# bjack205/altro

Hardware: AMD Instinct MI355X
Metric: iLQR backward+forward sweeps/sec (N knotpoints x batch) (higher is better)
Workload: dtype f64

## Files before the change

### altro_amd/__init__.py

```python
import ctypes as C
import os

import numpy as np

_HERE = os.path.dirname(os.path.abspath(__file__))
LIB_PATH = os.path.join(_HERE, "lib", "libaltro_hip.so")

F64, F32 = 0, 1
PLAN_AUTO, PLAN_GENERIC, PLAN_MFMA16, PLAN_LANE, PLAN_MFMA32 = 0, 1, 2, 3, 4
STORE_QBLOCKS = 0x1
LANE_FUSED = 0x4
F32_PURE = 0x2
TILE_USER_BLOCKS = 0x2
GENERIC_MATRIX_CORES = 0x8
TVLQR_SUCCESS = -1

C_ABI_SYMBOLS = [
    "altro_hip_version", "altro_hip_last_error", "altro_hip_device_count", "altro_hip_device_info", "altro_hip_device_pci_bus_id",
    "altro_hip_batch_create", "altro_hip_batch_create_dims", "altro_hip_batch_destroy", "altro_hip_batch_plan",
    "altro_hip_batch_device_bytes", "altro_hip_set_dynamics", "altro_hip_set_cost",
    "altro_hip_set_initial_state", "altro_hip_set_host_batch", "altro_hip_backward", "altro_hip_forward_ltv", "altro_hip_sweep",
    "altro_hip_synchronize", "altro_hip_get_K", "altro_hip_get_d", "altro_hip_get_P",
    "altro_hip_get_p", "altro_hip_get_x", "altro_hip_get_u", "altro_hip_get_y",
    "altro_hip_get_delta_V", "altro_hip_get_status", "altro_hip_get_qblocks",
    "altro_hip_stats_reduce", "altro_hip_comm_unique_id", "altro_hip_comm_create", "altro_hip_comm_create_all",
    "altro_hip_comm_destroy", "altro_hip_comm_rank", "altro_hip_comm_world", "altro_hip_comm_device", "altro_hip_stats_allreduce", "altro_hip_stats_allreduce_multi",
    "altro_hip_profile_enable", "altro_hip_profile_reset",
    "altro_hip_profile_get", "altro_hip_profile_get_range", "altro_hip_profile_dropped", "altro_hip_algorithmic_bytes",
    "altro_hip_set_model", "altro_hip_set_model_source", "altro_hip_model_row_layout", "altro_hip_set_tracking_cost", "altro_hip_set_quadratic_cost",
    "altro_hip_set_input_guess", "altro_hip_set_state_guess",
    "altro_hip_open_loop_rollout", "altro_hip_accept", "altro_hip_expand", "altro_hip_merit",
    "altro_hip_stationarity", "altro_hip_get_nominal", "altro_hip_get_expansion",
    "altro_hip_default_solve_options", "altro_hip_set_forms", "altro_hip_get_forms", "altro_hip_ilqr_solve", "altro_hip_last_solve_counts",
    "altro_hip_ilqr_solve_async", "altro_hip_ilqr_poll", "altro_hip_ilqr_wait",
    "altro_hip_linesearch_host",
    "altro_hip_add_linear_constraint", "altro_hip_add_user_constraint", "altro_hip_clear_constraints", "altro_hip_reset_duals",
    "altro_hip_get_duals", "altro_hip_set_duals", "altro_hip_get_penalty", "altro_hip_set_penalty", "altro_hip_shift_duals", "altro_hip_feasibility",
    "altro_hip_shift_trajectory", "altro_hip_update_linear_costs", "altro_hip_get_knot",
    "altro_hip_set_pointer_mode",
]
CONE_EQUALITY, CONE_IDENTITY, CONE_INEQUALITY, CONE_SOC = 0, 1, 2, 3

DUAL_TAIL_KEEP, DUAL_TAIL_ZERO = 0, 1
FORM_NO_SPECULATION, FORM_NO_RUNAHEAD, FORM_NO_MERIT2, FORM_MERIT_LDS, FORM_MERIT_DPP_ALWAYS = 0x1, 0x2, 0x4, 0x8, 0x10
FORM_EXPAND_LDS, FORM_ALROWS_LDS, FORM_ROLLOUT_ROUNDS, FORM_SEQUENCED, FORM_MERIT_ONE_LAUNCH = 0x20, 0x40, 0x80, 0x100, 0x200
FORM_LANE_QUAD_OFF, FORM_LANE_QUAD_ON, FORM_GENERIC_LATE_Q_OFF, FORM_GENERIC_LATE_Q_ON, FORM_FUSED_CLOCK = 0x400, 0x800, 0x1000, 0x2000, 0x4000
FORM_AFFINE_EXACT = 0x8000
FORM_NO_COMPACTION = 0x10000
FORM_GENERIC_MERIT_LDS = 0x20000


def forms_from_env():
    e = os.environ
    off = lambda name: e.get(name) is not None and e[name].strip() not in ("",) and _atoi(e[name]) == 0
    f = 0
    if "ALTRO_HIP_NO_SPECULATION" in e: f |= FORM_NO_SPECULATION
    if "ALTRO_HIP_NO_RUNAHEAD" in e and not off("ALTRO_HIP_NO_RUNAHEAD"): f |= FORM_NO_RUNAHEAD
    if off("ALTRO_HIP_MERIT2"): f |= FORM_NO_MERIT2
    if off("ALTRO_HIP_MERIT_DPP"): f |= FORM_MERIT_LDS
    elif e.get("ALTRO_HIP_MERIT_DPP") is not None and _atoi(e["ALTRO_HIP_MERIT_DPP"]) == 2: f |= FORM_MERIT_DPP_ALWAYS
    if off("ALTRO_HIP_EXPAND_DPP"): f |= FORM_EXPAND_LDS
    if off("ALTRO_HIP_ALROWS_DPP"): f |= FORM_ALROWS_LDS
    if off("ALTRO_HIP_AFFINE"): f |= FORM_ROLLOUT_ROUNDS
    if off("ALTRO_HIP_FUSED") or "ALTRO_HIP_NO_FUSED" in e: f |= FORM_SEQUENCED
    if off("ALTRO_HIP_MERIT_SPLIT"): f |= FORM_MERIT_ONE_LAUNCH
    if "ALTRO_HIP_LANE_QUAD" in e: f |= FORM_LANE_QUAD_OFF if _atoi(e["ALTRO_HIP_LANE_QUAD"]) == 0 else FORM_LANE_QUAD_ON
    if "ALTRO_HIP_GENERIC_LATE_Q" in e: f |= FORM_GENERIC_LATE_Q_OFF if _atoi(e["ALTRO_HIP_GENERIC_LATE_Q"]) == 0 else FORM_GENERIC_LATE_Q_ON
    if "ALTRO_HIP_FUSED_CLOCK" in e: f |= FORM_FUSED_CLOCK
    if "ALTRO_HIP_AFFINE_EXACT" in e: f |= FORM_AFFINE_EXACT
    if "ALTRO_HIP_NO_COMPACTION" in e: f |= FORM_NO_COMPACTION
    return f


def _atoi(text):
    try:
        return int(text.strip() or 0)
    except ValueError:
        return 0

MODEL_LINEAR, MODEL_DOUBLE_INTEGRATOR, MODEL_PENDULUM, MODEL_BICYCLE, MODEL_USER, MODEL_QUADROTOR, MODEL_QUADROTOR13 = 0, 1, 2, 3, 4, 5, 6
MERIT_FN = C.CFUNCTYPE(None, C.c_double, C.POINTER(C.c_double), C.POINTER(C.c_double), C.c_void_p)


class SolveOptions(C.Structure):
    _fields_ = [("iterations_max", C.c_int), ("tol_stationarity", C.c_double),
                ("tol_primal_feasibility", C.c_double), ("tol_meritfun_gradient", C.c_double),
                ("use_backtracking_linesearch", C.c_int), ("penalty_initial", C.c_double),
                ("penalty_scaling", C.c_double), ("penalty_max", C.c_double), ("reg_initial", C.c_double),
                ("reg_retry_max", C.c_int), ("reg_scale", C.c_double), ("reg_min", C.c_double),
                ("reg_max", C.c_double), ("stop_when_running_at_most", C.c_int),
                ("forms", C.c_uint), ("fused_sweeps", C.c_int), ("decision_margin", C.c_double)]


class SolveResult(C.Structure):
    _fields_ = [("status", C.c_int), ("iterations", C.c_int), ("stationarity", C.c_double),
                ("final_alpha", C.c_double), ("final_phi", C.c_double), ("primal_feasibility", C.c_double),
                ("penalty", C.c_double), ("dual_updates", C.c_int), ("reg_retries", C.c_int)]


class PollRecord(C.Structure):
    _fields_ = [("result", SolveResult), ("u0", C.c_double * 4), ("done", C.c_int), ("reserved", C.c_int)]


class AltroHipError(RuntimeError):
    pass


class Stats(C.Structure):
    _fields_ = [("problems", C.c_int64), ("cholesky_failures", C.c_int64), ("converged", C.c_int64),
                ("iterations", C.c_int64), ("sum_cost", C.c_double),
                ("sum_delta_V0", C.c_double), ("sum_delta_V1", C.c_double),
                ("max_stationarity", C.c_double), ("max_feasibility", C.c_double), ("max_abs_xN", C.c_double),
                ("non_finite", C.c_int64)]
    SUM_FIELDS = ("problems", "cholesky_failures", "converged", "iterations", "sum_cost", "sum_delta_V0", "sum_delta_V1",
                  "non_finite")
    MAX_FIELDS = ("max_stationarity", "max_feasibility", "max_abs_xN")

    def as_dict(self):
        return {k: getattr(self, k) for k, _ in self._fields_}


COMM_ID_BYTES = 128

# ... 516 lines not shown
```

### altro_amd/csrc/capi_ilqr.hip

```cpp
#include "capi_internal.h"

#include <cstring>

using namespace altro_hip;
using namespace altro_hip::capi;

namespace altro_hip {
namespace capi {

static AlInput al_input(const altro_hip_batch* h) {
  return AlInput{h->plan, h->n, h->m, h->N, h->batch, h->dtype == ALTRO_HIP_F64 ? sizeof(double) : sizeof(float), h->ragged, h->nxv, h->nuv,
                 h->al_defs, h->al_knots, h->al_G, h->al_g};
}
static int al_copy(altro_hip_batch* h, void** dst, const void* src, size_t bytes) {
  if (const int rc = dmalloc(h, dst, bytes)) return rc;
  HIP_TRY(hipMemcpy(*dst, src, bytes, hipMemcpyHostToDevice));
  return 0;
}
static int al_copy_pool(altro_hip_batch* h, void** dst, const std::vector<double>& pool) {
  if (h->dtype == ALTRO_HIP_F64) return al_copy(h, dst, pool.data(), pool.size() * sizeof(double));
  const std::vector<float> f = al_pool_as<float>(pool);
  return al_copy(h, dst, f.data(), f.size() * sizeof(float));
}
static int al_upload_tables(altro_hip_batch* h) {
// ... 124 lines not shown
    const RouteStep& st = route.step[i];
    a.mode = st.mode; a.mp.kind = st.kind;
    if (st.rtc) {
      if (!module_current) {
        if (const int rc = rtc_current(h, shape)) return rc;
        module_current = true;
      }
      if (const int rc = rtc_step(h, st, &a)) return rc;
      continue;
    }
    const int rc = launch_step(h, st, a);
    if (rc == 1) return fail(ALTRO_HIP_ERR_UNSUPPORTED, "internal error: kernel %#x is not in its launcher unit", st.id);
    if (rc) return fail(ALTRO_HIP_ERR_HIP, "iLQR kernel launch failed");
  }
  return 0;
}
template <typename T>
int lane_run(altro_hip_batch* h, int which, bool use_alpha, bool use_active, int want_deriv, double alpha_const, int mode) {
  const IlqrArgs<T> a = ilqr_args<T>(h, use_alpha, use_active, want_deriv, alpha_const);
  const RouteShape shape = route_shape(h);
  const Route route = loop_route(shape, RouteCall{which, mode, a.spec_trials});
  if (route.error == ROUTE_NO_MODEL) return fail(ALTRO_HIP_ERR_UNSUPPORTED, "no device model for (kind, n, m) = (%d, %d, %d)", h->model.kind, h->n, h->m);
  if (route.error) return fail(ALTRO_HIP_ERR_UNSUPPORTED, "operation %d is not available on plan LANE", which);
  return route_execute(h, shape, route, a);
}
template <typename S>
int wave_run(altro_hip_batch* h, int which, bool use_alpha, bool use_active, int want_deriv, double alpha_const, int mode) {
  IlqrWaveArgs<S> a;
  a.al = al_table<S>(h);
  a.mode = mode;
  const bool user_al = a.al.enabled && h->al_sum.has_user;
  if (user_al && (h->forms & (ALTRO_HIP_FORM_MERIT_LDS | ALTRO_HIP_FORM_ALROWS_LDS | ALTRO_HIP_FORM_EXPAND_LDS)))
    return fail(ALTRO_HIP_ERR_UNSUPPORTED, "constraint blocks from source on plan MFMA16 run in the row-layout kernels only: the LDS comparison forms "
                                           "(ALTRO_HIP_FORM_MERIT_LDS, _ALROWS_LDS, _EXPAND_LDS) do not evaluate them");
  a.penalty_scaling = h->expand_penalty_scaling; a.penalty_max = h->expand_penalty_max;
  a.costd = (const S*)h->m_costd; a.costd_term = (const S*)h->m_costd_term; a.cost_dense = h->cost_dense ? 1 : 0;
  if (h->model_set) a.mp = h->model;
  a.dyn = (const S*)h->m_in; a.dyn_bs = h->m_st.in_bs; a.dyn_ks = h->m_st.in_ks;
  a.cin = (S*)h->m_cin; a.cin_bs = h->m_st.cin_bs; a.cin_ks = h->m_st.cin_ks;
  a.term = (S*)h->m_term; a.out = (const S*)h->m_out; a.out_bs = h->m_st.out_bs; a.out_ks = h->m_st.out_ks;
  a.outn = (const S*)h->m_outn; a.nom = (S*)h->m_nom; a.cand = (S*)h->m_xuy; a.xuy_bs = h->m_st.xuy_bs;
  a.xuy_ks = h->m_st.xuy_ks; a.costp = (const S*)h->m_costp; a.x0 = (const S*)h->x0;
  a.alpha = use_alpha ? h->i_alpha : nullptr; a.active = use_active ? h->i_active : nullptr;
  a.phi = h->i_phi; a.dphi = h->i_dphi; a.prob = h->i_prob; a.N = h->N; a.batch = h->batch;
  a.want_derivative = want_deriv; a.alpha_const = alpha_const;
  a.cand_spec = (S*)h->i_cand_spec; a.spec_trials = h->i_cand_spec ? h->spec_trials : 1; a.spec_sel = h->i_spec_sel;
  a.spec_pre = h->i_cand_spec ? h->spec_pre : 0;
  a.spec_stride = (int64_t)h->batch * (h->N + 1) * MF_XUY;
  a.ls_beta = h->spec_beta; a.ls_max_iters = h->spec_max_iters;
  a.skip = which == IK_STATIONARITY ? h->stat_skip : nullptr;
  const bool aff_on = sizeof(S) == 8 && h->aff_enabled && !h->model_set;
  const bool aff_store = aff_on && h->aff_store && (which == IK_MERIT2 || which == IK_MERIT);
  const RouteShape shape = route_shape(h);
  const Route route = loop_route(shape, RouteCall{which, mode, a.spec_trials, aff_on && !aff_store && which == IK_MERIT && h->aff_round && !a.spec_pre});
  if (route.error) return fail(ALTRO_HIP_ERR_UNSUPPORTED, "operation %d is not available on plan MFMA16", which);
  if constexpr (sizeof(S) == 8) {
    a.aff = route.count && (route.step[0].id & KF_AFF) ? 1 : 0;
    if (aff_store || a.aff) { a.sens = (double*)h->i_sens; a.sens_alpha = (double*)h->i_sens_alpha; }
    if (a.aff) { a.aff_part = (double*)h->i_aff_part; a.aff_on = (int*)h->i_aff_on; }
  }
  return route_execute(h, shape, route, a);
}
struct GenSizes { int64_t sx, su, sQ, sR, sH; };
GenSizes gen_sizes(const altro_hip_batch* h) {
  GenSizes z{0, 0, 0, 0, 0};
  for (int k = 0; k <= h->N; ++k) {
    const int64_t nk = h->ragged ? h->nxv[k] : h->n, mk = k < h->N ? (h->ragged ? h->nuv[k] : h->m) : 0;
    z.sx += nk; z.su += mk; z.sQ += nk * nk; z.sR += mk * mk; z.sH += mk * nk;
  }
  return z;
}
template <typename T>
int gen_run(altro_hip_batch* h, int which, bool use_alpha, bool use_active, int want_deriv, double alpha_const, int mode) {
  const int n = h->n, m = h->m, N = h->N;
  IlqrGenArgs<T> a;
  a.A = (const T*)h->g_arr[G_A]; a.A_bs = h->g_bstride[G_A]; a.B = (const T*)h->g_arr[G_B]; a.B_bs = h->g_bstride[G_B];
  a.f = (const T*)h->g_arr[G_f]; a.f_bs = h->g_bstride[G_f];
  a.Q = (T*)h->g_arr[G_Q]; a.Q_bs = h->g_bstride[G_Q]; a.R = (T*)h->g_arr[G_R]; a.R_bs = h->g_bstride[G_R];
  a.H = (T*)h->g_arr[G_H]; a.H_bs = h->g_bstride[G_H]; a.q = (T*)h->g_arr[G_q]; a.q_bs = h->g_bstride[G_q];
  a.r = (T*)h->g_arr[G_r]; a.r_bs = h->g_bstride[G_r];
  a.K = (const T*)h->g_arr[G_K]; a.K_bs = h->g_bstride[G_K]; a.d = (const T*)h->g_arr[G_d]; a.d_bs = h->g_bstride[G_d];
  a.P = (const T*)h->g_arr[G_P]; a.P_bs = h->g_bstride[G_P]; a.p = (const T*)h->g_arr[G_p]; a.p_bs = h->g_bstride[G_p];
  a.x = (T*)h->g_arr[G_x]; a.x_bs = h->g_bstride[G_x]; a.u = (T*)h->g_arr[G_u]; a.u_bs = h->g_bstride[G_u];
  a.y = (T*)h->g_arr[G_y]; a.y_bs = h->g_bstride[G_y];
  a.xn = (T*)h->g_xn; a.un = (T*)h->g_un;
  a.cQ = (const T*)h->g_cQ; a.cR = (const T*)h->g_cR; a.cH = (const T*)h->g_cH; a.cq = (const T*)h->g_cq; a.cr = (const T*)h->g_cr;
  a.cc = (const T*)h->g_cc;
  a.x0 = (const T*)h->x0; a.x0_stride = h->x0_stride;
  a.alpha = use_alpha ? h->i_alpha : nullptr; a.active = use_active ? h->i_active : nullptr; a.alpha_const = alpha_const;
  a.phi = h->i_phi; a.dphi = h->i_dphi; a.prob = h->i_prob;
  a.N = N; a.n = n; a.m = m; a.batch = h->batch; a.want_derivative = want_deriv; a.mode = mode;
  a.off = h->g_off; a.nx = h->g_nx; a.nu = h->g_nu;
  const GenSizes gs = gen_sizes(h);
  a.sx = gs.sx; a.su = gs.su; a.sQ = gs.sQ; a.sR = gs.sR; a.sH = gs.sH;
  a.al = al_table<T>(h);
  const RouteShape shape = route_shape(h);
  a.row32 = row32_eligible(shape) ? 1 : 0;
  a.row32m = row32_model_eligible(shape) ? 1 : 0;
  if ((a.row32 || a.row32m) && which == IK_STATIONARITY && N > R32_STAT_CHUNK) {
    const size_t need = (size_t)((N + R32_STAT_CHUNK - 1) / R32_STAT_CHUNK) * h->batch * 2 * sizeof(double);
    if (h->g_stat_part_bytes < need) {
      if (h->g_stat_part) { (void)hipFree(h->g_stat_part); h->g_stat_part = nullptr; h->g_stat_part_bytes = 0; }
      if (hipMalloc((void**)&h->g_stat_part, need) == hipSuccess) h->g_stat_part_bytes = need;
      else { (void)hipGetLastError(); h->g_stat_part = nullptr; }
    }
    a.stat_part = h->g_stat_part;
  }
// ... 802 lines not shown
```

### altro_amd/csrc/ilqr_launch_mfma16.hip

```cpp
#include <hip/hip_runtime.h>

#include "kernels/ilqr_mfma16.hip"
#include "kernels/ilqr_merit2_dpp.hip"
#include "loop_route.h"

namespace altro_hip {

using namespace capi;

#define GO(...) hipLaunchKernelGGL((__VA_ARGS__), grid, block, st.lds, stream, a); break
#define MERIT(DUAL_, DENSE_, AFF_)                                                                                              \
  case merit_id(true, DUAL_, DENSE_, false, AFF_): GO(wave_merit_dpp_kernel<S, true, DUAL_, DENSE_, 0, false, AFF_>);           \
  case merit_id(true, DUAL_, DENSE_, true, AFF_): GO(wave_merit_dpp_kernel<S, true, DUAL_, DENSE_, 0, true, AFF_>);             \
  case merit_id(false, DUAL_, DENSE_, true, AFF_): GO(wave_merit_dpp_kernel<S, false, DUAL_, DENSE_, 0, true, AFF_>)

template <typename S>
static int wave_launch(hipStream_t stream, const RouteStep& st, const IlqrWaveArgs<S>& a) {
  const dim3 grid(st.gx, st.gy, st.gz), block(st.block);
  if constexpr (sizeof(S) == 8) {
    if ((st.id & KF_AFF) || st.id == K_WAVE_AFF_REDUCE) {
      switch (st.id) {
        MERIT(false, false, true);
        MERIT(false, true, true);
        case K_WAVE_AFF_REDUCE: hipLaunchKernelGGL(wave_aff_reduce_kernel<S>, grid, block, 0, stream, a, st.chunks); break;
        default: return 1;
      }
      return hipGetLastError() == hipSuccess ? 0 : 2;
    }
  }
  switch (st.id) {
    case K_WAVE_ROLLOUT: GO(wave_rollout_kernel<S>);
    case K_WAVE_ACCEPT: GO(wave_accept_kernel<S>);
    case K_WAVE_EXPAND_DPP | KF_DENSE: GO(wave_expand_dpp_kernel<S, true>);
    case K_WAVE_EXPAND_DPP | KF_ALLSEL: GO(wave_expand_dpp_kernel<S, false, true>);
    case K_WAVE_EXPAND_DPP: GO(wave_expand_dpp_kernel<S, false>);
    case K_WAVE_EXPAND_LDS: GO(wave_expand_kernel<S>);
    case K_WAVE_EXPAND_GRAD | KF_DENSE: GO(wave_expand_grad_dense_kernel<S>);
    case K_WAVE_EXPAND_GRAD: GO(wave_expand_grad_kernel<S>);
    case K_WAVE_DUAL_DPP: GO(wave_dual_update_dpp_kernel<S>);
    case K_WAVE_DUAL_LDS: GO(wave_dual_update_kernel<S>);
    MERIT(false, false, false);
    MERIT(false, true, false);
    MERIT(true, false, false);
    MERIT(true, true, false);
    case K_WAVE_MERIT_LDS | KF_AL: GO(wave_merit_kernel<S, true>);
    case K_WAVE_MERIT_LDS: GO(wave_merit_kernel<S, false>);
    case K_WAVE_SPEC_SELECT: GO(wave_spec_select_kernel<S>);
    case K_WAVE_STATIONARITY: GO(wave_stationarity_kernel<S>);
    case K_WAVE_FEAS_DPP: GO(wave_feasibility_dpp_kernel<S>);
    case K_WAVE_SHIFT: GO(wave_shift_kernel<S>);
    default: return 1;
  }
  return hipGetLastError() == hipSuccess ? 0 : 2;
}
#undef MERIT
#undef GO
template <>
int ilqr_wave_launch_kernel<double>(hipStream_t stream, const RouteStep& st, const IlqrWaveArgs<double>& a) { return wave_launch<double>(stream, st, a); }
template <>
int ilqr_wave_launch_kernel<float>(hipStream_t stream, const RouteStep& st, const IlqrWaveArgs<float>& a) { return wave_launch<float>(stream, st, a); }

}
```

### altro_amd/csrc/kernels/ilqr_merit2_dpp.hip

```cpp
#pragma once

namespace altro_hip {

constexpr int MD_ZLD = 18;
constexpr int MD_OUT0 = 12 * MD_ZLD;
constexpr int MD_F0 = MD_OUT0 + MF_OUT;
constexpr int MD_NOM0 = MD_F0 + 12;
constexpr int MD_CP0 = MD_NOM0 + MF_NOM;
constexpr int MD_IMG = MD_CP0 + MF_COSTP;
constexpr int MD_IMG_DENSE = MD_CP0 + MF_COST;
static_assert(MF_DYN % 2 == 0 && MF_OUT % 2 == 0 && MF_NOM % 2 == 0 && MF_COSTP % 2 == 0 && MD_IMG % 2 == 0, "records move as pairs");

typedef double md_d2 __attribute__((ext_vector_type(2)));
typedef float md_f2 __attribute__((ext_vector_type(2)));
template <typename S> struct md_pair_of;
template <> struct md_pair_of<double> { typedef md_d2 type; };
template <> struct md_pair_of<float> { typedef md_f2 type; };
template <typename S>
__device__ __forceinline__ md_d2 md_ld(const S* __restrict__ p, int pair) {
  const typename md_pair_of<S>::type v = *reinterpret_cast<const typename md_pair_of<S>::type*>(p + 2 * pair);
  return md_d2{(double)v[0], (double)v[1]};
}
template <bool DENSE = false>
struct MeritPairRegs { md_d2 z[3], f, o[3], nm, cp[DENSE ? 3 : 1]; };
// ... 1008 lines not shown
      else a.cin[(size_t)b * a.cin_bs + (size_t)k * a.cin_ks + MF_OFF_HR + (r - 12) * 16 + j] = (S)v;
    }
  }
}

template <typename S>
__global__ __launch_bounds__(64) void wave_dual_update_dpp_kernel(IlqrWaveArgs<S> a) {
  const int lane = threadIdx.x, j = lane & 15;
  const int wpk = (a.batch + 3) >> 2;
  const int k = (int)(blockIdx.x / wpk), b0 = (int)(blockIdx.x % wpk) * 4, b_own = b0 + (lane >> 4);
  if (k > a.N || !a.al.enabled) return;
  const bool on = b_own < a.batch && a.prob[b_own < a.batch ? b_own : 0].dual != 0;
  const unsigned long long onm = __ballot(on);
  if (onm == 0ull) return;
  const int b = on ? b_own : b0 + (__builtin_ctzll(onm) >> 4);
  const bool terminal = k == a.N;
  const S* c = a.cand + (size_t)b * a.xuy_bs + (size_t)k * a.xuy_ks;
  const double w = j < 12 ? (double)c[j] : (terminal ? 0.0 : (double)c[12 + j]);
  double jvr[AL_TILE_MAXC], cost = 0.0, viol = 0.0;
#ifdef MD_USER_BLOCKS
  __shared__ double uimg[4][MD_UIMG_ROW];
  dpp_al_rows<S, true>(a.al, k, b, a.batch, w, terminal, a.prob[b].rho_est, j, jvr, cost, viol, on, uimg[lane >> 4]);
#else
  dpp_al_rows<S, true>(a.al, k, b, a.batch, w, terminal, a.prob[b].rho_est, j, jvr, cost, viol, on);
#endif
}
template <typename S>
__global__ __launch_bounds__(64) void wave_feasibility_dpp_kernel(IlqrWaveArgs<S> a) {
  const int lane = threadIdx.x, j = lane & 15;
  const int wpk = (a.batch + 3) >> 2;
  const int k = (int)(blockIdx.x / wpk), b0 = (int)(blockIdx.x % wpk) * 4, b_own = b0 + (lane >> 4);
  if (k > a.N) return;
  bool on = b_own < a.batch;
  if (on && a.active && !a.active[b_own]) on = false;
  if (on && a.skip && a.skip[b_own]) on = false;
  const unsigned long long onm = __ballot(on);
  if (onm == 0ull) return;
  const int b = on ? b_own : b0 + (__builtin_ctzll(onm) >> 4);
  const bool terminal = k == a.N;
  const S* c = a.cand + (size_t)b * a.xuy_bs + (size_t)k * a.xuy_ks;
  const double w = j < 12 ? (double)c[j] : (terminal ? 0.0 : (double)c[12 + j]);
  double jvr[AL_TILE_MAXC], cost = 0.0, viol = 0.0;
#ifdef MD_USER_BLOCKS
  __shared__ double uimg[4][MD_UIMG_ROW];
  dpp_al_rows<S>(a.al, k, b, a.batch, w, terminal, a.prob[b].rho, j, jvr, cost, viol, false, uimg[lane >> 4]);
#else
  dpp_al_rows<S>(a.al, k, b, a.batch, w, terminal, a.prob[b].rho, j, jvr, cost, viol);
#endif
#pragma unroll
  for (int o = 8; o > 0; o >>= 1) viol = fmax(viol, __shfl_xor(viol, o, 64));
  if (j == 0 && on && viol > 0.0)
    atomicMax(reinterpret_cast<unsigned long long*>(&a.prob[b].feasibility), (unsigned long long)__double_as_longlong(viol));
}


}
```

### altro_amd/csrc/loop_route.h

```cpp
#pragma once
#include <algorithm>
#include <cstdint>

#include "al_tables.h"
#include "kernels/ilqr_types.h"
#include "rtc_unit.h"

namespace altro_hip {
namespace capi {

enum KernelId : int {
  KF_AL = 1,
  KF_DUAL = 2,
  KF_DENSE = 4,
  KF_SOC = 8,
  KF_AFF = 16,
  KF_WIDE = 32,
  KF_MODEL = 64,
  KF_ALLSEL = 128,
  KF_STAGED = 128,
  KF_MASK = 255,
  K_WAVE_ROLLOUT = 1 << 8 , K_WAVE_ACCEPT = 2 << 8,
  K_WAVE_EXPAND_GRAD = 3 << 8,
  K_WAVE_EXPAND_DPP = 4 << 8 , K_WAVE_EXPAND_LDS = 5 << 8,
// ... 15 lines not shown
#define ILQR_LANE_MODELS(X)                                                                 \
  X(MODEL_PENDULUM, 2, 1) X(MODEL_BICYCLE, 4, 2) X(MODEL_DOUBLE_INTEGRATOR, 2, 1)           \
  X(MODEL_DOUBLE_INTEGRATOR, 4, 2) X(MODEL_DOUBLE_INTEGRATOR, 6, 3)
constexpr bool lane_model_supported(int kind, int n, int m) {
#define X(K_, N_, M_) if (kind == K_ && n == N_ && m == M_) return true;
  ILQR_LANE_MODELS(X)
#undef X
  return false;
}
constexpr int merit_id(bool al, bool dual, bool dense, bool soc, bool aff = false, int more = 0) {
  return K_WAVE_MERIT_DPP | (al ? KF_AL : 0) | (dual ? KF_DUAL : 0) | (dense ? KF_DENSE : 0) | (soc ? KF_SOC : 0) | (aff ? KF_AFF : 0) | more;
}
enum RouteUnit { RU_MFMA16, RU_MFMA16_MODEL, RU_MFMA16_WIDE, RU_LANE, RU_GENERIC, RU_ROW32 , RU_ROW32_MODEL };
constexpr int route_unit(int id) {
  return id >= K_LANE ? RU_LANE : id >= K_ROW_MERIT ? ((id & KF_MODEL) ? RU_ROW32_MODEL : RU_ROW32) : id >= K_GEN_ROLLOUT ? RU_GENERIC : (id & KF_WIDE) ? RU_MFMA16_WIDE : (id & KF_MODEL) ? RU_MFMA16_MODEL : RU_MFMA16;
}
constexpr int route_rtc_slot(int id) {
  if (id >= K_LANE) return (id - K_LANE) >> 8;
  switch (id & ~KF_MASK) {
    case K_WAVE_ROLLOUT: return RTT_ROLLOUT;
    case K_WAVE_EXPAND_DYN: return RTT_EXPAND_DYN;
    case K_WAVE_MERIT_DPP: return (id & KF_DUAL) ? RTT_MERIT2 : RTT_MERIT;
    case K_WAVE_EXPAND_DPP: return RTT_EXPAND_AL;
    case K_WAVE_DUAL_DPP: return RTT_DUAL;
    case K_WAVE_FEAS_DPP: return RTT_FEAS;
    case K_GEN_ROLLOUT: return RTG_ROLLOUT;
    case K_GEN_EXPAND_DYN: return RTG_EXPAND_DYN;
    case K_GEN_MERIT: return RTG_MERIT;
    case K_ROW_MERIT: return (id & KF_DUAL) ? RTG_ROW_MERIT2 : RTG_ROW_MERIT;
    case K_ROW_EXPAND_DYN: return RTG_ROW_EXPAND_DYN;
    case K_GEN_STATIONARITY: return RTG_STATIONARITY;
    case K_GEN_EXPAND_AL: return RTG_EXPAND_AL;
    case K_GEN_DUAL: return RTG_DUAL;
    default: return -1;
  }
}

struct RouteShape {
  int plan;
  bool f64, ragged;
  int n, m, N, batch;
  int model;
  bool cost_dense;
  bool merit_split;
  unsigned forms;
  bool al_enabled;
  AlSummary al;
  bool row_ok;
};
struct RouteCall {
  int which, mode, spec_trials;
  bool aff;
  bool stat_part;
};
enum RouteError { ROUTE_OK = 0, ROUTE_NO_KERNEL , ROUTE_NO_MODEL  };
struct RouteStep {
  bool rtc;
  int id;
  unsigned gx, gy, gz, block, lds;
  int mode, kind;
  int chunks;
};
constexpr int ROUTE_MAX_STEPS = 4;
struct Route {
  int error = ROUTE_OK, count = 0;
  RouteStep step[ROUTE_MAX_STEPS] = {};
};

inline unsigned route_merit_lds(const RouteShape& s, bool rtc) {
  if (!s.al_enabled) return 0u;
  const unsigned padded = (unsigned)s.al.Gpad_count * 8u;
  return rtc && s.al.has_user ? std::max(padded, (unsigned)AL_GP_DEF * 8u) : padded;
}
inline int route_tile_module_key(const RouteShape& s) {
  return (s.al_enabled ? 1 : 0) | (s.cost_dense ? 2 : 0) | ((s.al_enabled && s.al.max_ncon > AL_MAXC) ? 4 : 0) | ((s.al_enabled && s.al.has_user) ? 8 : 0);
}

inline Route route_mfma16(const RouteShape& s, const RouteCall& c) {
  Route r;
  const auto frm = [&](unsigned bit) { return (s.forms & bit) != 0; };
  const bool al = s.al_enabled, wide = al && s.al.max_ncon > AL_MAXC, model = s.model != MODEL_LINEAR, user = s.model == MODEL_USER;
  const bool user_al = user && al && s.al.has_user;
  const int dense = s.cost_dense ? KF_DENSE : 0;
  int mode = c.mode;
  if (c.which == IK_STATIONARITY || c.which == IK_DUAL) mode = frm(ALTRO_HIP_FORM_ALROWS_LDS) ? 0 : STAT_NO_FEAS;
  if (c.which == IK_EXPAND && frm(ALTRO_HIP_FORM_EXPAND_LDS) && !s.cost_dense) mode |= EXPAND_LDS;
  if (model && c.which == IK_EXPAND && (mode & EXPAND_GRADIENT) && !(mode & EXPAND_NEXT)) mode |= EXPAND_DYN;
  if (c.which == IK_MERIT) mode = frm(ALTRO_HIP_FORM_MERIT_LDS) ? 0 : frm(ALTRO_HIP_FORM_MERIT_DPP_ALWAYS) ? 3 : 2;
  const int lib_kind = user ? (int)MODEL_LINEAR : s.model;
  int rtc_kind = MODEL_USER;
  const auto add = [&](bool rtc, int id, int64_t gx, unsigned gy = 1, unsigned gz = 1, unsigned block = 64, unsigned lds = 0, int chunks = 0) {
    r.step[r.count++] = RouteStep{rtc, id, (unsigned)gx, gy, gz, block, lds, mode, rtc ? rtc_kind : lib_kind, chunks};
  };
  const auto no_kernel = [&] { r.error = ROUTE_NO_KERNEL; r.count = 0; return r; };
  if (model && (!s.f64 || (!user && s.model != MODEL_QUADROTOR))) return no_kernel();
  if (wide && !s.f64 && (c.which == IK_EXPAND || c.which == IK_MERIT || c.which == IK_MERIT2)) return no_kernel();
  const int64_t knots = (int64_t)s.N + 1, rows4 = (s.batch + 3) / 4, flat = ((int64_t)s.batch * knots * 16 + 255) / 256;
  const unsigned waves = (unsigned)mf_grid(s.batch), pairs = (unsigned)mf_grid((s.batch + 1) / 2);
  const unsigned trials = (unsigned)std::max(c.spec_trials, 1);
  switch (c.which) {
    case IK_ROLLOUT:
      if (model) add(user, K_WAVE_ROLLOUT | KF_MODEL, rows4);
      else add(false, K_WAVE_ROLLOUT, waves);
      break;
    case IK_ACCEPT: add(false, K_WAVE_ACCEPT, std::min<int64_t>(flat, 1 << 20), 1, 1, 256); break;
    case IK_EXPAND:
      if (model && (mode & EXPAND_DYN)) add(user, K_WAVE_EXPAND_DYN | KF_MODEL, rows4 * s.N);
      if (user_al) {
        add(true, K_WAVE_EXPAND_DPP | dense | (wide ? KF_WIDE : 0), rows4 * knots);
        break;
      }
      if (al && (wide || dense || !(mode & EXPAND_LDS))) add(false, K_WAVE_EXPAND_DPP | (wide ? KF_WIDE : 0) | (dense ? dense : s.al.all_sel ? KF_ALLSEL : 0), rows4 * knots);
      else if (al) add(false, K_WAVE_EXPAND_LDS, s.batch * knots);
      else if (mode & EXPAND_GRADIENT) add(false, K_WAVE_EXPAND_GRAD | dense, std::min<int64_t>(flat, 262144), 1, 1, 256);
      break;
    case IK_DUAL:
      if (user_al) { add(true, K_WAVE_DUAL_DPP, rows4 * knots); break; }
      if (mode & STAT_NO_FEAS) add(false, K_WAVE_DUAL_DPP, rows4 * knots);
      else add(false, K_WAVE_DUAL_LDS, s.batch * knots);
      break;
    case IK_MERIT:
    case IK_MERIT2: {
      const bool dual = c.which == IK_MERIT2, aff = !dual && !model && s.f64 && c.aff && mode >= 2;
      const unsigned gy = dual ? 1u : (trials + 1) / 2;
      if (!model && !wide && !dual && !aff && !dense && mode != 2 && mode != 3) {
        add(false, K_WAVE_MERIT_LDS | (al ? KF_AL : 0), waves, trials);
        break;
      }
      const int id = merit_id(al, dual, s.cost_dense, model || !al || s.al.has_soc, aff, (model ? KF_MODEL : 0) | (wide ? KF_WIDE : 0));
      if (aff) {
        const int chunks = (s.N + MD_AFF_CHUNK - 1) / MD_AFF_CHUNK;
        add(false, id, pairs, gy, (unsigned)chunks, 64, route_merit_lds(s, false));
        add(false, K_WAVE_AFF_REDUCE | (wide ? KF_WIDE : 0), ((int64_t)ILQR_SPEC_TRIALS * s.batch + 255) / 256, 1, 1, 256, 0, chunks);
      } else {
        add(user, id, pairs, gy, 1, 64, route_merit_lds(s, user));
      }
      break;
    }
    case IK_SPEC_SELECT: add(false, K_WAVE_SPEC_SELECT, s.batch); break;
    case IK_STATIONARITY:
      if (user_al) { mode |= STAT_FEAS_USER; rtc_kind = MODEL_LINEAR; }
      if (al && (mode & STAT_NO_FEAS)) {
        add(false, K_WAVE_STATIONARITY, waves);
        add(user_al, K_WAVE_FEAS_DPP, rows4 * knots);
      } else {
        mode &= ~STAT_NO_FEAS;
        add(false, K_WAVE_STATIONARITY, waves);
      }
      break;
    case IK_SHIFT: add(false, K_WAVE_SHIFT, ((int64_t)s.batch * 16 + 255) / 256, 1, 1, 256); break;
    default: return no_kernel();
  }
  return r;
}

inline Route route_lane(const RouteShape& s, const RouteCall& c) {
  Route r;
  const bool user = s.model == MODEL_USER;
  if (!user && !lane_model_supported(s.model, s.n, s.m)) { r.error = ROUTE_NO_MODEL; return r; }
  const auto add = [&](int slot, bool dense, int64_t gx, unsigned gy, unsigned block) {
    r.step[r.count++] = RouteStep{user, lane_id(slot, dense), (unsigned)gx, gy, 1, block, 0, c.mode, s.model, 0};
  };
  const int64_t total = (int64_t)s.batch * (s.N + 1), lanes = (s.batch + 63) / 64;
  const int64_t flat = std::min<int64_t>((total + 255) / 256, 1 << 20), flat64 = std::min<int64_t>((total + 63) / 64, 1 << 20);
  const unsigned trials = (unsigned)std::max(c.spec_trials, 1);
  switch (c.which) {
    case IK_ROLLOUT: add(RTC_ROLLOUT, false, lanes, 1, 64); break;
    case IK_ACCEPT: add(RTC_ACCEPT, false, flat, 1, 256); break;
    case IK_EXPAND: add(RTC_EXPAND, s.cost_dense, flat64, 1, 64); break;
    case IK_MERIT:
      if (s.merit_split) {
        add(RTC_MERIT_ROLL, false, lanes, trials, 64);
        add(RTC_MERIT_POINT, s.cost_dense, flat64, trials, 64);
        add(RTC_MERIT_SUM, false, lanes, trials, 64);
      } else {
        add(RTC_MERIT, s.cost_dense, lanes, trials, 64);
      }
      break;
    case IK_SPEC_SELECT: add(RTC_SPEC_SELECT, false, flat, 1, 256); break;
    case IK_DUAL: add(RTC_DUAL, false, flat, 1, 256); break;
    case IK_SHIFT: add(RTC_SHIFT, false, std::min<int64_t>(((int64_t)s.batch * (s.n + s.m) + 255) / 256, 1 << 20), 1, 256); break;
    case IK_STATIONARITY:
      add(RTC_ZERO_RESIDUALS, false, (s.batch + 255) / 256, 1, 256);
      add(RTC_STATIONARITY, false, flat64, 1, 64);
      break;
    default: r.error = ROUTE_NO_KERNEL;
  }
  return r;
}

constexpr bool tile32_shape_ok(int n, int m) { return n >= 5 && n <= T32_MAX_N && m >= 1 && m <= T32_MAX_M && n + m <= 32 && !(n <= 12 && m <= 4); }
constexpr bool gen_model_supported(int kind, int n, int m) { return kind == MODEL_QUADROTOR13 && n == 13 && m == 4; }
inline bool row32_shape(const RouteShape& s) {
  return s.plan == ALTRO_HIP_PLAN_GENERIC && s.f64 && !s.ragged && tile32_shape_ok(s.n, s.m) && !(s.forms & ALTRO_HIP_FORM_GENERIC_MERIT_LDS) && (!s.al_enabled || s.al.row32_ok);
}
inline bool row32_eligible(const RouteShape& s) { return row32_shape(s) && s.model == MODEL_LINEAR; }
inline bool row32_model_eligible(const RouteShape& s) {
// ... 19 lines not shown
  const int64_t b = s.batch, knots = (int64_t)s.N + 1, pairs = (b + 1) / 2, flat = std::min<int64_t>((b * knots * (s.n + s.m) + 255) / 256, 1 << 20);
  const unsigned jv = al ? (unsigned)(GEN_AL_JV * sizeof(double)) : 0u;
  switch (c.which) {
    case IK_ROLLOUT:
      if (user || q13) add(user, K_GEN_ROLLOUT | KF_MODEL, (b + 63) / 64);
      else if (row32 && (mode & ROLLOUT_INIT)) add(false, K_ROW_INIT, pairs);
      else add(false, K_GEN_ROLLOUT, b);
      break;
    case IK_ACCEPT: add(false, K_GEN_ACCEPT, flat, 1, 256); break;
    case IK_EXPAND:
      if (user) kind = MODEL_LINEAR;
      if (user_al) add(true, K_GEN_EXPAND_AL, b * knots);
      else if (al && row32 && (!(mode & EXPAND_HESSIAN) || (mode & EXPAND_DIAG)) && !(mode & EXPAND_DYN)) add(false, K_ROW_EXPAND, pairs, (unsigned)((s.N + R32_EXPAND_CHUNK - 1) / R32_EXPAND_CHUNK));
      else if (al) add(false, K_GEN_EXPAND_AL, b * knots);
      else add(false, K_GEN_EXPAND, flat, 1, 256);
      kind = s.model;
      if ((user || q13) && (mode & EXPAND_DYN)) {
        if (row32m) add(user, K_ROW_EXPAND_DYN | KF_MODEL, (b * s.N + 1) / 2);
        else add(user, K_GEN_EXPAND_DYN | KF_MODEL, (b * s.N + 63) / 64);
      }
      break;
    case IK_DUAL: add(user_al, K_GEN_DUAL, b * knots); break;
    case IK_MERIT:
      if (user || q13) {
        if (row32m) add(user, K_ROW_MERIT | KF_MODEL, pairs);
        else add(user, K_GEN_MERIT | KF_MODEL, b, 1, 64, jv);
      } else if (row32) {
        add(false, K_ROW_MERIT, pairs);
      } else {
        const size_t stage = generic_merit_stage_elems(s.n, s.m) * (s.f64 ? 8 : 4);
        if (2560 + jv + stage <= 10 * 1024) add(false, K_GEN_MERIT | KF_STAGED, b, 1, 64, jv + (unsigned)stage);
        else add(false, K_GEN_MERIT, b, 1, 64, jv);
      }
      break;
    case IK_MERIT2:
      if (row32) add(false, K_ROW_MERIT | KF_DUAL, b);
      else if (row32m) add(user, K_ROW_MERIT | KF_DUAL | KF_MODEL, b);
      else r.error = ROUTE_NO_KERNEL;
      break;
    case IK_STATIONARITY:
      if (user_al) add(true, K_GEN_STATIONARITY, b);
      else if (row32 || row32m) {
        const int chunks = c.stat_part ? (s.N + R32_STAT_CHUNK - 1) / R32_STAT_CHUNK : 1;
        add(false, K_ROW_STAT, pairs, (unsigned)chunks);
        if (chunks > 1) add(false, K_ROW_STAT_REDUCE, (b + 255) / 256, 1, 256, 0, chunks);
      } else add(false, K_GEN_STATIONARITY, b);
      break;
    case IK_SHIFT: add(false, K_GEN_SHIFT, (b * (s.n + s.m) + 255) / 256, 1, 256); break;
    default: r.error = ROUTE_NO_KERNEL;
  }
  return r;
}

inline Route loop_route(const RouteShape& s, const RouteCall& c) {
  return s.plan == ALTRO_HIP_PLAN_GENERIC ? route_generic(s, c) : s.plan == ALTRO_HIP_PLAN_MFMA16 ? route_mfma16(s, c) : route_lane(s, c);
}

}

template <typename T> struct IlqrGenArgs;
template <typename S> int ilqr_wave_launch_kernel(hipStream_t stream, const capi::RouteStep& st, const IlqrWaveArgs<S>& a);
template <typename S> int ilqr_wave_launch_model(hipStream_t stream, const capi::RouteStep& st, const IlqrWaveArgs<S>& a);
template <typename S> int ilqr_wave_launch_wide(hipStream_t stream, const capi::RouteStep& st, const IlqrWaveArgs<S>& a);
template <typename T> int ilqr_launch_kernel(hipStream_t stream, const capi::RouteStep& st, int kind, int n, int m, const IlqrArgs<T>& a);
template <typename T> int ilqr_generic_launch(hipStream_t stream, const capi::RouteStep& st, const IlqrGenArgs<T>& a);
typedef int Row32Launch(hipStream_t stream, const capi::RouteStep& st, const IlqrGenArgs<double>& a);
Row32Launch row32_merit_unit0, row32_merit_unit1, row32_merit_unit2, row32_merit_unit3, row32_merit_unit4, row32_merit_unit5, row32_merit_unit6, row32_merit_unit7;
int row32_model_launch(hipStream_t stream, const capi::RouteStep& st, const IlqrGenArgs<double>& a);

}
```

### include/altro_hip/altro_hip.h

```cpp
#ifndef ALTRO_HIP_H_
#define ALTRO_HIP_H_

#include <stddef.h>
#include <stdint.h>

#ifdef __cplusplus
extern "C" {
#endif

#define ALTRO_HIP_VERSION 300
#define ALTRO_HIP_TVLQR_SUCCESS (-1)

typedef struct altro_hip_batch altro_hip_batch;

typedef enum altro_hip_dtype {
  ALTRO_HIP_F64 = 0,
  ALTRO_HIP_F32 = 1
} altro_hip_dtype;

typedef enum altro_hip_error {
  ALTRO_HIP_OK = 0,
  ALTRO_HIP_ERR_NO_DEVICE = -1,
  ALTRO_HIP_ERR_BAD_ARGUMENT = -2,
  ALTRO_HIP_ERR_UNSUPPORTED = -3,
// ... 89 lines not shown

int altro_hip_add_linear_constraint(altro_hip_batch* h, int k_first, int k_last, int cone, int p,
                                    const double* G, const double* g, int g_per_problem);
int altro_hip_clear_constraints(altro_hip_batch* h);
int altro_hip_reset_duals(altro_hip_batch* h, double penalty);
int altro_hip_get_duals(altro_hip_batch* h, int k, int slot, double* z );
enum { ALTRO_HIP_DUAL_TAIL_KEEP = 0, ALTRO_HIP_DUAL_TAIL_ZERO = 1 };
int altro_hip_set_duals(altro_hip_batch* h, int k, int slot, const double* z );
int altro_hip_get_penalty(altro_hip_batch* h, double* rho );
int altro_hip_set_penalty(altro_hip_batch* h, const double* rho, int batch_stride_zero);
int altro_hip_shift_duals(altro_hip_batch* h, int tail);
int altro_hip_feasibility(altro_hip_batch* h, double* out);

int altro_hip_shift_trajectory(altro_hip_batch* h);
int altro_hip_update_linear_costs(altro_hip_batch* h, const double* q, const double* r, const double* c,
                                  int k_first, int k_last, int kz, int bz);
int altro_hip_get_knot(altro_hip_batch* h, int k, double* x , double* u );

typedef struct altro_hip_solve_options {
  int iterations_max;
  double tol_stationarity;
  double tol_primal_feasibility;
  double tol_meritfun_gradient;
  int use_backtracking_linesearch;
  double penalty_initial;
  double penalty_scaling;
  double penalty_max;
  double reg_initial;
  int reg_retry_max;
  double reg_scale, reg_min, reg_max;
  int stop_when_running_at_most;
  unsigned forms;
  int fused_sweeps;
  double decision_margin;
} altro_hip_solve_options;
#define ALTRO_HIP_FORM_NO_SPECULATION 0x0001u
#define ALTRO_HIP_FORM_NO_RUNAHEAD 0x0002u
#define ALTRO_HIP_FORM_NO_MERIT2 0x0004u
#define ALTRO_HIP_FORM_MERIT_LDS 0x0008u
#define ALTRO_HIP_FORM_MERIT_DPP_ALWAYS 0x0010u
#define ALTRO_HIP_FORM_EXPAND_LDS 0x0020u
#define ALTRO_HIP_FORM_ALROWS_LDS 0x0040u
#define ALTRO_HIP_FORM_ROLLOUT_ROUNDS 0x0080u
#define ALTRO_HIP_FORM_SEQUENCED 0x0100u
#define ALTRO_HIP_FORM_MERIT_ONE_LAUNCH 0x0200u
#define ALTRO_HIP_FORM_LANE_QUAD_OFF 0x0400u
#define ALTRO_HIP_FORM_LANE_QUAD_ON 0x0800u
#define ALTRO_HIP_FORM_GENERIC_LATE_Q_OFF 0x1000u
#define ALTRO_HIP_FORM_GENERIC_LATE_Q_ON 0x2000u
#define ALTRO_HIP_FORM_AFFINE_EXACT 0x8000u
#define ALTRO_HIP_FORM_FUSED_CLOCK 0x4000u
#define ALTRO_HIP_FORM_NO_COMPACTION 0x10000u
#define ALTRO_HIP_FORM_GENERIC_MERIT_LDS 0x20000u
int altro_hip_set_forms(altro_hip_batch* h, unsigned forms);
unsigned altro_hip_get_forms(const altro_hip_batch* h);
typedef struct altro_hip_solve_result {
  int status;
  int iterations;
  double stationarity;
  double final_alpha;
  double final_phi;
  double primal_feasibility;
  double penalty;
  int dual_updates;
  int reg_retries;
} altro_hip_solve_result;
void altro_hip_default_solve_options(altro_hip_solve_options* opts);
int altro_hip_ilqr_solve(altro_hip_batch* h, const altro_hip_solve_options* opts,
                         altro_hip_solve_result* results);
int altro_hip_last_solve_counts(const altro_hip_batch* h, int* sweeps, int* merit_launches);

typedef struct altro_hip_poll_record {
  altro_hip_solve_result result;
  double u0[4];
  int done;
  int reserved;
} altro_hip_poll_record;
int altro_hip_ilqr_solve_async(altro_hip_batch* h, const altro_hip_solve_options* opts);
int altro_hip_ilqr_poll(altro_hip_batch* h, int* n_done, const altro_hip_poll_record** records);
int altro_hip_ilqr_wait(altro_hip_batch* h, altro_hip_solve_result* results);

typedef void (*altro_hip_merit_fn)(double alpha, double* phi, double* dphi, void* ctx);
double altro_hip_linesearch_host(altro_hip_merit_fn f, void* ctx, double alpha0, double phi0, double dphi0,
                                 int try_cubic_first, int use_backtracking, double c1, double c2,
                                 int* status, int* iters, double* phi, double* dphi);

typedef struct altro_hip_stats {
  int64_t problems;
  int64_t cholesky_failures;
  int64_t converged;
  int64_t iterations;
  double sum_cost;
  double sum_delta_V0;
  double sum_delta_V1;
  double max_stationarity;
  double max_feasibility;
  double max_abs_xN;
  int64_t non_finite;
} altro_hip_stats;
int altro_hip_stats_reduce(altro_hip_batch* h, altro_hip_stats* out);

typedef struct altro_hip_comm altro_hip_comm;
#define ALTRO_HIP_COMM_ID_BYTES 128
int altro_hip_comm_unique_id(void* id );
int altro_hip_comm_create(altro_hip_comm** out, int device, int rank, int world, const void* id);
int altro_hip_comm_create_all(altro_hip_comm** out , int ndev, const int* devices);
// ... 21 lines not shown
```

Before: 2.782 million.

## Walk several knots per wave in AL dual-update and feasibility DPP kernels

Adds walk variants of the MFMA16 augmented-Lagrangian dual-update and feasibility kernels. Each wave now processes a run of consecutive knots and prefetches the next knot's point, instead of launching one wave per knot. A heuristic picks the run length from batch and horizon, and new form bits can force one knot per wave or a specific run. This cuts the wave count and launch overhead and lets the feasibility max-reduction and atomic happen once per run, at the cost of less parallelism when grids are small. The metric measures backward+forward sweeps, which may not touch these AL kernels at all.

Result: slower. 2.707 million (-2.7%).

```diff
diff --git a/altro_amd/__init__.py b/altro_amd/__init__.py
--- a/altro_amd/__init__.py
+++ b/altro_amd/__init__.py
@@ -48,6 +48,11 @@
 FORM_AFFINE_EXACT = 0x8000
 FORM_NO_COMPACTION = 0x10000
 FORM_GENERIC_MERIT_LDS = 0x20000
+FORM_AL_ONE_KNOT = 0x40000
+
+
+def FORM_AL_RUN(n):
+    return (int(n) & 0xff) << 20
 
 
 def forms_from_env():
@@ -69,6 +74,8 @@
     if "ALTRO_HIP_FUSED_CLOCK" in e: f |= FORM_FUSED_CLOCK
     if "ALTRO_HIP_AFFINE_EXACT" in e: f |= FORM_AFFINE_EXACT
     if "ALTRO_HIP_NO_COMPACTION" in e: f |= FORM_NO_COMPACTION
+    if off("ALTRO_HIP_AL_WALK"): f |= FORM_AL_ONE_KNOT
+    if "ALTRO_HIP_AL_RUN" in e: f |= FORM_AL_RUN(_atoi(e["ALTRO_HIP_AL_RUN"]))
     return f
 
 
diff --git a/altro_amd/csrc/capi_ilqr.hip b/altro_amd/csrc/capi_ilqr.hip
--- a/altro_amd/csrc/capi_ilqr.hip
+++ b/altro_amd/csrc/capi_ilqr.hip
@@ -200,7 +200,8 @@
   const bool aff_on = sizeof(S) == 8 && h->aff_enabled && !h->model_set;
   const bool aff_store = aff_on && h->aff_store && (which == IK_MERIT2 || which == IK_MERIT);
   const RouteShape shape = route_shape(h);
-  const Route route = loop_route(shape, RouteCall{which, mode, a.spec_trials, aff_on && !aff_store && which == IK_MERIT && h->aff_round && !a.spec_pre});
+  const int walk = (h->forms & ALTRO_HIP_FORM_AL_ONE_KNOT) ? 0 : route_al_walk(h->batch, h->N, (int)ALTRO_HIP_FORM_AL_RUN_OF(h->forms));
+  const Route route = loop_route(shape, RouteCall{which, mode, a.spec_trials, aff_on && !aff_store && which == IK_MERIT && h->aff_round && !a.spec_pre, false, walk});
   if (route.error) return fail(ALTRO_HIP_ERR_UNSUPPORTED, "operation %d is not available on plan MFMA16", which);
   if constexpr (sizeof(S) == 8) {
     a.aff = route.count && (route.step[0].id & KF_AFF) ? 1 : 0;
diff --git a/altro_amd/csrc/ilqr_launch_mfma16.hip b/altro_amd/csrc/ilqr_launch_mfma16.hip
--- a/altro_amd/csrc/ilqr_launch_mfma16.hip
+++ b/altro_amd/csrc/ilqr_launch_mfma16.hip
@@ -27,6 +27,14 @@
       }
       return hipGetLastError() == hipSuccess ? 0 : 2;
     }
+  }
+  if (st.walk > 0) {
+    switch (st.id) {
+      case K_WAVE_DUAL_DPP: hipLaunchKernelGGL(wave_dual_update_walk_kernel<S>, grid, block, 0, stream, a, st.walk); break;
+      case K_WAVE_FEAS_DPP: hipLaunchKernelGGL(wave_feasibility_walk_kernel<S>, grid, block, 0, stream, a, st.walk); break;
+      default: return 1;
+    }
+    return hipGetLastError() == hipSuccess ? 0 : 2;
   }
   switch (st.id) {
     case K_WAVE_ROLLOUT: GO(wave_rollout_kernel<S>);
diff --git a/altro_amd/csrc/kernels/ilqr_merit2_dpp.hip b/altro_amd/csrc/kernels/ilqr_merit2_dpp.hip
--- a/altro_amd/csrc/kernels/ilqr_merit2_dpp.hip
+++ b/altro_amd/csrc/kernels/ilqr_merit2_dpp.hip
@@ -1084,6 +1084,58 @@
   if (j == 0 && on && viol > 0.0)
     atomicMax(reinterpret_cast<unsigned long long*>(&a.prob[b].feasibility), (unsigned long long)__double_as_longlong(viol));
 }
-
-
-}
+#ifndef MD_USER_BLOCKS
+template <typename S>
+__device__ __forceinline__ double walk_point_w(const IlqrWaveArgs<S>& a, int b, int k, int j) {
+  const S* c = a.cand + (size_t)b * a.xuy_bs + (size_t)k * a.xuy_ks;
+  const double wj = (double)c[j < 12 ? j : 12 + j];
+  return (j >= 12 && k == a.N) ? 0.0 : wj;
+}
+template <typename S>
+__global__ __launch_bounds__(64) void wave_dual_update_walk_kernel(IlqrWaveArgs<S> a, int run) {
+  const int lane = threadIdx.x, j = lane & 15;
+  const int k0 = (int)blockIdx.y * run, k1 = min(k0 + run, a.N + 1), b0 = (int)blockIdx.x * 4, b_own = b0 + (lane >> 4);
+  if (k0 >= k1 || !a.al.enabled) return;
+  const bool on = b_own < a.batch && a.prob[b_own < a.batch ? b_own : 0].dual != 0;
+  const unsigned long long onm = __ballot(on);
+  if (onm == 0ull) return;
+  const int b = on ? b_own : b0 + (__builtin_ctzll(onm) >> 4);
+  const double rho_est = a.prob[b].rho_est;
+  double w = walk_point_w(a, b, k0, j);
+#pragma unroll 1
+  for (int k = k0; k < k1; ++k) {
+    const double wn = walk_point_w(a, b, min(k + 1, k1 - 1), j);
+    double jvr[AL_TILE_MAXC], cost = 0.0, viol = 0.0;
+    dpp_al_rows<S, true>(a.al, k, b, a.batch, w, k == a.N, rho_est, j, jvr, cost, viol, on);
+    w = wn;
+  }
+}
+template <typename S>
+__global__ __launch_bounds__(64) void wave_feasibility_walk_kernel(IlqrWaveArgs<S> a, int run) {
+  const int lane = threadIdx.x, j = lane & 15;
+  const int k0 = (int)blockIdx.y * run, k1 = min(k0 + run, a.N + 1), b0 = (int)blockIdx.x * 4, b_own = b0 + (lane >> 4);
+  if (k0 >= k1) return;
+  bool on = b_own < a.batch;
+  if (on && a.active && !a.active[b_own]) on = false;
+  if (on && a.skip && a.skip[b_own]) on = false;
+  const unsigned long long onm = __ballot(on);
+  if (onm == 0ull) return;
+  const int b = on ? b_own : b0 + (__builtin_ctzll(onm) >> 4);
+  const double rho = a.prob[b].rho;
+  double w = walk_point_w(a, b, k0, j), viol = 0.0;
+#pragma unroll 1
+  for (int k = k0; k < k1; ++k) {
+    const double wn = walk_point_w(a, b, min(k + 1, k1 - 1), j);
+    double jvr[AL_TILE_MAXC], cost = 0.0;
+    dpp_al_rows<S>(a.al, k, b, a.batch, w, k == a.N, rho, j, jvr, cost, viol);
+    w = wn;
+  }
+#pragma unroll
+  for (int o = 8; o > 0; o >>= 1) viol = fmax(viol, __shfl_xor(viol, o, 64));
+  if (j == 0 && on && viol > 0.0)
+    atomicMax(reinterpret_cast<unsigned long long*>(&a.prob[b].feasibility), (unsigned long long)__double_as_longlong(viol));
+}
+#endif
+
+
+}
diff --git a/altro_amd/csrc/loop_route.h b/altro_amd/csrc/loop_route.h
--- a/altro_amd/csrc/loop_route.h
+++ b/altro_amd/csrc/loop_route.h
@@ -91,6 +91,7 @@
   int which, mode, spec_trials;
   bool aff;
   bool stat_part;
+  int walk = 0;
 };
 enum RouteError { ROUTE_OK = 0, ROUTE_NO_KERNEL , ROUTE_NO_MODEL  };
 struct RouteStep {
@@ -99,6 +100,7 @@
   unsigned gx, gy, gz, block, lds;
   int mode, kind;
   int chunks;
+  int walk = 0;
 };
 constexpr int ROUTE_MAX_STEPS = 4;
 struct Route {
@@ -132,6 +134,12 @@
     r.step[r.count++] = RouteStep{rtc, id, (unsigned)gx, gy, gz, block, lds, mode, rtc ? rtc_kind : lib_kind, chunks};
   };
   const auto no_kernel = [&] { r.error = ROUTE_NO_KERNEL; r.count = 0; return r; };
+  const auto add_al = [&](int id, int64_t rows4, int64_t knots) {
+    if (c.walk > 0) {
+      add(false, id, rows4, (unsigned)((knots + c.walk - 1) / c.walk));
+      r.step[r.count - 1].walk = c.walk;
+    } else add(false, id, rows4 * knots);
+  };
   if (model && (!s.f64 || (!user && s.model != MODEL_QUADROTOR))) return no_kernel();
   if (wide && !s.f64 && (c.which == IK_EXPAND || c.which == IK_MERIT || c.which == IK_MERIT2)) return no_kernel();
   const int64_t knots = (int64_t)s.N + 1, rows4 = (s.batch + 3) / 4, flat = ((int64_t)s.batch * knots * 16 + 255) / 256;
@@ -155,7 +163,7 @@
       break;
     case IK_DUAL:
       if (user_al) { add(true, K_WAVE_DUAL_DPP, rows4 * knots); break; }
-      if (mode & STAT_NO_FEAS) add(false, K_WAVE_DUAL_DPP, rows4 * knots);
+      if (mode & STAT_NO_FEAS) add_al(K_WAVE_DUAL_DPP, rows4, knots);
       else add(false, K_WAVE_DUAL_LDS, s.batch * knots);
       break;
     case IK_MERIT:
@@ -181,7 +189,8 @@
       if (user_al) { mode |= STAT_FEAS_USER; rtc_kind = MODEL_LINEAR; }
       if (al && (mode & STAT_NO_FEAS)) {
         add(false, K_WAVE_STATIONARITY, waves);
-        add(user_al, K_WAVE_FEAS_DPP, rows4 * knots);
+        if (user_al) add(true, K_WAVE_FEAS_DPP, rows4 * knots);
+        else add_al(K_WAVE_FEAS_DPP, rows4, knots);
       } else {
         mode &= ~STAT_NO_FEAS;
         add(false, K_WAVE_STATIONARITY, waves);
@@ -307,6 +316,14 @@
   return r;
 }
 
+constexpr int AL_WALK_MAX = 16, AL_WALK_WAVES = 65536;
+inline int route_al_walk(int batch, int N, int forced = 0) {
+  const int64_t knots = (int64_t)N + 1, rows4 = (batch + 3) / 4;
+  const int64_t least = (knots + 65534) / 65535;
+  if (forced > 0) return (int)std::max<int64_t>(least, std::min<int64_t>(forced, knots));
+  return (int)std::max<int64_t>(least, std::min<int64_t>(std::min<int64_t>(AL_WALK_MAX, knots), rows4 * knots / AL_WALK_WAVES));
+}
+
 inline Route loop_route(const RouteShape& s, const RouteCall& c) {
   return s.plan == ALTRO_HIP_PLAN_GENERIC ? route_generic(s, c) : s.plan == ALTRO_HIP_PLAN_MFMA16 ? route_mfma16(s, c) : route_lane(s, c);
 }
diff --git a/include/altro_hip/altro_hip.h b/include/altro_hip/altro_hip.h
--- a/include/altro_hip/altro_hip.h
+++ b/include/altro_hip/altro_hip.h
@@ -165,6 +165,9 @@
 #define ALTRO_HIP_FORM_FUSED_CLOCK 0x4000u
 #define ALTRO_HIP_FORM_NO_COMPACTION 0x10000u
 #define ALTRO_HIP_FORM_GENERIC_MERIT_LDS 0x20000u
+#define ALTRO_HIP_FORM_AL_ONE_KNOT 0x40000u
+#define ALTRO_HIP_FORM_AL_RUN(n) (((unsigned)(n) & 0xffu) << 20)
+#define ALTRO_HIP_FORM_AL_RUN_OF(forms) (((forms) >> 20) & 0xffu)
 int altro_hip_set_forms(altro_hip_batch* h, unsigned forms);
 unsigned altro_hip_get_forms(const altro_hip_batch* h);
 typedef struct altro_hip_solve_result {
```
